# yjh0410/YOLO-Nano

Measured on AMD Instinct MI355X. Metric: images/sec YOLO-Nano-1.0x 416x416 bs=32 inference (network + decode + NMS + host delivery), higher is better.
Workload: dtype f32 (split-f16 MFMA x3, fp32 accumulate); 1 GPU; YOLO-Nano-1.0x 416x416 bs=32/GPU fp32 inference, COCO 80-class head + NMS (BASELINE configs[1]); inputs resident in HBM, kept detections delivered to pinned host memory inside the timed region; global_batch=32, parallelism=image-sharded x1, no collective, rccl_ranks=1, launch_mode=eager, streams_per_gpu=4

## Files before the change

### yolo-nano_amd/csrc/kernels_conv.hip

```cpp
#include "yn_internal.h"
#include "yn_device.h"

#include <cstdio>
#include <mutex>
#include <set>
#include <string>

namespace ynk {

static thread_local const char* g_last_kernel = "";
const char* last_kernel_name() { return g_last_kernel; }
void set_last_kernel_name(const char* n) { g_last_kernel = n; }

bool g_log_lds = getenv("YN_LOG_LDS") != nullptr && atoi(getenv("YN_LOG_LDS")) != 0;
void note_launch_lds(const char* kernel, size_t dyn_lds, unsigned threads)
{
    static std::mutex mu;
    static std::set<std::string> seen;
    char line[512];
    snprintf(line, sizeof line, "yn_lds %s %zu %u", kernel, dyn_lds, threads);
    std::lock_guard<std::mutex> lk(mu);
    if (seen.insert(line).second) fprintf(stderr, "%s\n", line);
}

// ... 1008 lines not shown
static int choose_pw_cfg(int M, int K, int Npad)
{
    const int nt32 = Npad / 32;
    auto pick_nt = [&](int wn, int maxnt) {
        const int need = (nt32 + wn - 1) / wn;
        if (need <= maxnt) return need;
        for (int nt = maxnt; nt >= 1; --nt) if (nt32 % (nt * wn) == 0) return nt;
        return maxnt;
    };
    auto blocks = [&](int wm, int wn, int nt) {
        const long BM = 32 * wm, BN = 32 * nt * wn;
        return ((M + BM - 1) / BM) * ((Npad + BN - 1) / BN);
    };
    int wm = 4, wn = 1, nt = pick_nt(1, 4);
    if (blocks(wm, wn, nt) < 384) {
        const int nt2 = pick_nt(2, 2);
        if (blocks(2, 2, nt2) > blocks(wm, wn, nt)) { wm = 2; wn = 2; nt = nt2; }
        if (blocks(wm, wn, nt) < 256) {
            const int nt3 = pick_nt(4, 2);
            if (blocks(1, 4, nt3) > blocks(wm, wn, nt)) { wm = 1; wn = 4; nt = nt3; }
            if (blocks(wm, wn, nt) < 256 && nt > 1 && blocks(wm, wn, 1) > blocks(wm, wn, nt)) nt = 1;
        }
    }
    const bool one_shot = K <= 64;
    int idx = find_pw_cfg(wm, wn, nt, one_shot ? 32 : 16, one_shot ? 1 : 2);
    const TileCfg& c = g_pw_cfgs[idx];
    if (c.WM != wm || c.WN != wn || c.NT != nt) idx = find_pw_cfg(wm, wn, nt, 16, 2);
    return idx;
}

void launch_pw(const GemmArgs& a, hipStream_t s)
{
    int idx = a.cfg;
    if (idx == N_PW_CFGS + N_PWD_CFGS + N_PWS_CFGS) { if (launch_pw_pipe(a, s)) return; idx = -1; }
    if (a.Wsh && (idx < 0 || idx >= N_PW_CFGS + N_PWD_CFGS) && launch_pw_split(a, idx < 0 ? -1 : idx - N_PW_CFGS - N_PWD_CFGS, s)) return;
    if (idx >= N_PW_CFGS + N_PWD_CFGS) idx = -1;
    if (idx >= N_PW_CFGS && idx < N_PW_CFGS + N_PWD_CFGS && launch_pw_direct(a, idx - N_PW_CFGS, s)) return;
    if (idx < 0 || idx >= N_PW_CFGS) idx = choose_pw_cfg(a.M, a.K, a.Npad);
    const TileCfg& c = g_pw_cfgs[idx];
    const int BM = 32 * c.WM, BN = 32 * c.NT * c.WN;
    dim3 grid(xcd_grid((a.M + BM - 1) / BM) * ((a.Npad + BN - 1) / BN));
    g_last_kernel = g_pw_names[idx];
    int i = 0;
#define X(wm, wn, nt, kp, nb)                                                                              \
    if (i++ == idx) { hipLaunchKernelGGL((gemm_conv_kernel<wm, wn, nt, 0, kp, nb>), grid, dim3(256), 0, s, a); return; }
    YN_PW_CONFIGS(X)
#undef X
}

static void launch_gemm_3x3(const GemmArgs& a, hipStream_t s)
{
    const int nt32 = a.Npad / 32;
    if (nt32 % 3 == 0) {
        dim3 grid(xcd_grid((a.M + 127) / 128) * (a.Npad / 96));
        g_last_kernel = "gemm_conv_kernel<4,1,3,1,16,2>";
        hipLaunchKernelGGL((gemm_conv_kernel<4, 1, 3, 1, 16, 2>), grid, dim3(256), 0, s, a);
    } else {
        dim3 grid(xcd_grid((a.M + 127) / 128) * nt32);
        g_last_kernel = "gemm_conv_kernel<4,1,1,1,16,2>";
        hipLaunchKernelGGL((gemm_conv_kernel<4, 1, 1, 1, 16, 2>), grid, dim3(256), 0, s, a);
    }
}

void launch_conv3x3(const GemmArgs& a, hipStream_t s)
{
    const int nt32 = a.Npad / 32;
    const int NT = nt32 >= 3 && nt32 % 3 == 0 ? 3 : (nt32 % 2 == 0 ? 2 : 1);
    if (a.Wsh && a.Wsl && a.K == 96 && a.Npad == 96 && a.in_off == 0 && a.in_ld == 96 && (a.N & 3) == 0 && (a.out_ld & 3) == 0 && (a.out_off & 3) == 0 &&
        conv3x3_split_lds(a.W, 1, 1) <= 160 * 1024) {
        static unsigned long long attr_s = 0;
        if (attr_pending(attr_s)) {
            (void)hipFuncSetAttribute(reinterpret_cast<const void*>(conv3x3_split_kernel<3, 2>), hipFuncAttributeMaxDynamicSharedMemorySize, 160 * 1024);
            (void)hipFuncSetAttribute(reinterpret_cast<const void*>(conv3x3_split_kernel<1, 2, 1>), hipFuncAttributeMaxDynamicSharedMemorySize, 160 * 1024);
            (void)hipFuncSetAttribute(reinterpret_cast<const void*>(conv3x3_split_kernel<1, 1, 9>), hipFuncAttributeMaxDynamicSharedMemorySize, 160 * 1024);
            (void)hipFuncSetAttribute(reinterpret_cast<const void*>(conv3x3_split_kernel<1, 1, 3>), hipFuncAttributeMaxDynamicSharedMemorySize, 160 * 1024);
            (void)hipFuncSetAttribute(reinterpret_cast<const void*>(conv3x3_split_kernel<1, 1, 1>), hipFuncAttributeMaxDynamicSharedMemorySize, 160 * 1024);
        }
        const int tiles = (a.M + 127) / 128;
        if (tiles >= 256) {
            g_last_kernel = "conv3x3_split_kernel<3,2>";
            hipLaunchKernelGGL((conv3x3_split_kernel<3, 2>), dim3(xcd_grid(tiles), 1), dim3(256), conv3x3_split_lds(a.W, 3, 2), s, a);
        } else if (tiles * 3 >= 256) {
            g_last_kernel = "conv3x3_split_kernel<1,2>";
            hipLaunchKernelGGL((conv3x3_split_kernel<1, 2, 1>), dim3(xcd_grid(tiles), 3), dim3(256), conv3x3_split_lds(a.W, 1, 2, 1), s, a);
        } else if (conv3x3_split_lds(a.W, 1, 1, 9) <= 160 * 1024) {
            g_last_kernel = "conv3x3_split_kernel<1,1,9>";
            hipLaunchKernelGGL((conv3x3_split_kernel<1, 1, 9>), dim3(xcd_grid(tiles), 3), dim3(256), conv3x3_split_lds(a.W, 1, 1, 9), s, a);
        } else if (conv3x3_split_lds(a.W, 1, 1, 3) <= 160 * 1024) {
            g_last_kernel = "conv3x3_split_kernel<1,1,3>";
            hipLaunchKernelGGL((conv3x3_split_kernel<1, 1, 3>), dim3(xcd_grid(tiles), 3), dim3(256), conv3x3_split_lds(a.W, 1, 1, 3), s, a);
        } else {
            g_last_kernel = "conv3x3_split_kernel<1,1,1>";
            hipLaunchKernelGGL((conv3x3_split_kernel<1, 1, 1>), dim3(xcd_grid(tiles), 3), dim3(256), conv3x3_split_lds(a.W, 1, 1, 1), s, a);
        }
        return;
    }
    if (a.K == 96 && NT == 3 && a.in_off == 0 && a.in_ld == 96 && (a.N & 3) == 0 && (a.out_ld & 3) == 0 && (a.out_off & 3) == 0 &&
        conv3x3_halo_tap_lds(a.W, 96, 3) <= 160 * 1024) {
        static unsigned long long attr_t = 0;
        if (attr_pending(attr_t)) {
            (void)hipFuncSetAttribute(reinterpret_cast<const void*>(conv3x3_halo_tap_kernel<3, 96, 1>), hipFuncAttributeMaxDynamicSharedMemorySize, 160 * 1024);
            (void)hipFuncSetAttribute(reinterpret_cast<const void*>(conv3x3_halo_tap_kernel<1, 96, 1>), hipFuncAttributeMaxDynamicSharedMemorySize, 160 * 1024);
            (void)hipFuncSetAttribute(reinterpret_cast<const void*>(conv3x3_halo_tap_kernel<1, 96, 2>), hipFuncAttributeMaxDynamicSharedMemorySize, 160 * 1024);
        }
        const int tiles = (a.M + 127) / 128;
        if (tiles * (a.Npad / 96) >= 256) {
            g_last_kernel = "conv3x3_halo_tap_kernel<3,96,1>";
            hipLaunchKernelGGL((conv3x3_halo_tap_kernel<3, 96, 1>), dim3(xcd_grid(tiles), a.Npad / 96), dim3(256), conv3x3_halo_tap_lds(a.W, 96, 3), s, a);
        } else if (conv3x3_halo_tap_lds(a.W, 96, 1) > 80 * 1024 && conv3x3_halo_tap_lds(a.W, 96, 1, 2) <= 80 * 1024) {
            g_last_kernel = "conv3x3_halo_tap_kernel<1,96,2>";
            hipLaunchKernelGGL((conv3x3_halo_tap_kernel<1, 96, 2>), dim3(xcd_grid(tiles), a.Npad / 32), dim3(256), conv3x3_halo_tap_lds(a.W, 96, 1, 2), s, a);
        } else {
            g_last_kernel = "conv3x3_halo_tap_kernel<1,96,1>";
            hipLaunchKernelGGL((conv3x3_halo_tap_kernel<1, 96, 1>), dim3(xcd_grid(tiles), a.Npad / 32), dim3(256), conv3x3_halo_tap_lds(a.W, 96, 1), s, a);
        }
        return;
    }
    const size_t lds = (a.K % 32 == 0 && a.in_off == 0) ? conv3x3_halo_lds(a.W, a.K, NT) : (size_t)1 << 30;
    if (lds <= 160 * 1024 && a.K / 2 <= 256) {
        static unsigned long long attr = 0;
        if (attr_pending(attr)) {
            (void)hipFuncSetAttribute(reinterpret_cast<const void*>(conv3x3_halo_kernel<1>), hipFuncAttributeMaxDynamicSharedMemorySize, 160 * 1024);
            (void)hipFuncSetAttribute(reinterpret_cast<const void*>(conv3x3_halo_kernel<2>), hipFuncAttributeMaxDynamicSharedMemorySize, 160 * 1024);
            (void)hipFuncSetAttribute(reinterpret_cast<const void*>(conv3x3_halo_kernel<3>), hipFuncAttributeMaxDynamicSharedMemorySize, 160 * 1024);
        }
        dim3 grid((a.M + 127) / 128, a.Npad / (32 * NT));
        if (NT == 3) { g_last_kernel = "conv3x3_halo_kernel<3>"; hipLaunchKernelGGL(conv3x3_halo_kernel<3>, grid, dim3(256), lds, s, a); }
        else if (NT == 2) { g_last_kernel = "conv3x3_halo_kernel<2>"; hipLaunchKernelGGL(conv3x3_halo_kernel<2>, grid, dim3(256), lds, s, a); }
        else { g_last_kernel = "conv3x3_halo_kernel<1>"; hipLaunchKernelGGL(conv3x3_halo_kernel<1>, grid, dim3(256), lds, s, a); }
        return;
    }
    launch_gemm_3x3(a, s);
}

template <int STRIDE, int VEC, int R>
__device__ __forceinline__ void dwconv3x3_block(const DwArgs& a, unsigned bid, unsigned nblocks)
{
    typedef typename VecT<VEC>::type vec;
    constexpr int NCOL = STRIDE == 1 ? R + 2 : 2 * R + 1;
    const int Ho = (a.H - 1) / STRIDE + 1, Wo = (a.W - 1) / STRIDE + 1;
    const int cv_n = a.C / VEC, segs = (Wo + R - 1) / R;
    const int total = a.B * Ho * segs * cv_n;
    const int i = xcd_block(bid, nblocks) * 256 + threadIdx.x;
    if (i >= total) return;
    const int cv = i % cv_n;
    int q = i / cv_n;
    const int seg = q % segs; q /= segs;
    const int oy = q % Ho, b = q / Ho;
    const int c = cv * VEC, ox0 = seg * R;
    vec col[3][NCOL];
#pragma unroll
    for (int ky = 0; ky < 3; ++ky) {
        const int iy = oy * STRIDE - 1 + ky;
        const bool yok = iy >= 0 && iy < a.H;
        const float* row = a.in + ((size_t)(b * a.H + (yok ? iy : 0)) * a.W) * a.in_ld + a.in_off + c;
#pragma unroll
        for (int j = 0; j < NCOL; ++j) {
            const int ix = ox0 * STRIDE - 1 + j;
            const unsigned mk = opaque_mask(yok && ix >= 0 && ix < a.W);
            col[ky][j] = vmask(*reinterpret_cast<const vec*>(row + (size_t)(ix < 0 ? 0 : (ix >= a.W ? a.W - 1 : ix)) * a.in_ld), mk);
        }
    }
    vec w[9];
#pragma unroll
    for (int k = 0; k < 9; ++k) w[k] = *reinterpret_cast<const vec*>(a.w + k * a.C + c);
    const vec bias = *reinterpret_cast<const vec*>(a.bias + c);
    float* orow = a.out + ((size_t)(b * Ho + oy) * Wo) * a.out_ld + a.out_off + c;
#pragma unroll
    for (int o = 0; o < R; ++o) {
        if (ox0 + o >= Wo) break;
        vec acc = bias;
#pragma unroll
        for (int ky = 0; ky < 3; ++ky)
#pragma unroll
            for (int kx = 0; kx < 3; ++kx) vfma(acc, col[ky][o * STRIDE + kx], w[ky * 3 + kx]);
        *reinterpret_cast<vec*>(orow + (size_t)(ox0 + o) * a.out_ld) = vact(acc, a.act);
    }
}

template <int STRIDE, int VEC, int R>
__global__ __launch_bounds__(256) void dwconv3x3_kernel(DwArgs a) { dwconv3x3_block<STRIDE, VEC, R>(a, blockIdx.x, gridDim.x); }

template <int R>
__global__ __launch_bounds__(256) void dwconv3x3_group_kernel(Group<DwArgs> g)
{
    unsigned local, nb;
    const int p = group_problem(g.first, blockIdx.x, local, nb);
    dwconv3x3_block<1, 4, R>(g.a[p], local, nb);
}

bool dw_group_ok(const DwArgs* a, int n)
{
    if (n < 1 || n > YN_GROUP_MAX) return false;
    for (int p = 0; p < n; ++p)
        if (a[p].stride != 1 || (a[p].C % 4) || (a[p].in_ld % 4) || (a[p].in_off % 4) || (a[p].out_ld % 4) || (a[p].out_off % 4)) return false;
    return true;
}

void launch_dw_group(const DwArgs* a, int n, hipStream_t s)
{
    auto blocks_for = [&](const DwArgs& q, int r) { return (unsigned)(((long)q.B * q.H * ((q.W + r - 1) / r) * (q.C / 4) + 255) / 256); };
    unsigned all4 = 0;
    for (int p = 0; p < n; ++p) all4 += blocks_for(a[p], 4);
    const int R = all4 >= 1024 ? 4 : 2;
    Group<DwArgs> g{};
    unsigned tot = 0;
    for (int p = 0; p < YN_GROUP_MAX; ++p) {
        g.first[p] = tot;
        if (p < n) { g.a[p] = a[p]; tot += xcd_grid(blocks_for(a[p], R)); }
    }
    g.first[YN_GROUP_MAX] = tot;
    if (R == 4) { g_last_kernel = "dwconv3x3_group_kernel<4>"; hipLaunchKernelGGL(dwconv3x3_group_kernel<4>, dim3(tot), dim3(256), 0, s, g); }
    else        { g_last_kernel = "dwconv3x3_group_kernel<2>"; hipLaunchKernelGGL(dwconv3x3_group_kernel<2>, dim3(tot), dim3(256), 0, s, g); }
}

void launch_dw(const DwArgs& a, hipStream_t s)
{
    const int Ho = (a.H - 1) / a.stride + 1, Wo = (a.W - 1) / a.stride + 1;
    const bool v4 = (a.C % 4 == 0) && (a.in_ld % 4 == 0) && (a.in_off % 4 == 0) && (a.out_ld % 4 == 0) && (a.out_off % 4 == 0);
    auto blocks_for = [&](int vec, int r) { return ((long)a.B * Ho * ((Wo + r - 1) / r) * (a.C / vec) + 255) / 256; };
#define YN_DW(ST, V, R) { g_last_kernel = "dwconv3x3_kernel<" #ST "," #V "," #R ">"; \
        hipLaunchKernelGGL((dwconv3x3_kernel<ST, V, R>), dim3(xcd_grid((unsigned)blocks_for(V, R))), dim3(256), 0, s, a); return; }
    if (a.stride == 1) {
        if (v4) { if (blocks_for(4, 4) >= 1024) YN_DW(1, 4, 4) else YN_DW(1, 4, 2) }
        else    { if (blocks_for(2, 8) >= 1024) YN_DW(1, 2, 8) else YN_DW(1, 2, 4) }
    } else {
        if (v4) { if (blocks_for(4, 4) >= 1024) YN_DW(2, 4, 4) else YN_DW(2, 4, 2) }
        else    { if (blocks_for(2, 4) >= 1024) YN_DW(2, 2, 4) else YN_DW(2, 2, 2) }
    }
#undef YN_DW
}

template <int COUT>
__global__ __launch_bounds__(256) void stem_kernel(const float* __restrict__ x, int B, int H, int W,
                                                    const float* __restrict__ w, const float* __restrict__ bias,
                                                    int act, float* __restrict__ y)
{
    __shared__ __attribute__((aligned(16))) float ws[28 * COUT];
    for (int i = threadIdx.x; i < 27 * COUT; i += 256) ws[i] = w[i];
    for (int i = threadIdx.x; i < COUT; i += 256) ws[27 * COUT + i] = bias[i];
    __syncthreads();
    const int Ho = (H - 1) / 2 + 1, Wo = (W - 1) / 2 + 1, Wp = (Wo + 1) / 2;
    const long total = (long)B * Ho * Wp;
    const long p = (long)blockIdx.x * 256 + threadIdx.x;
    if (p >= total) return;
    const int opx = (int)(p % Wp);
    const long q = p / Wp;
    const int oy = (int)(q % Ho);
    const int b = (int)(q / Ho);
    const int ox0 = opx * 2;
    const bool has1 = ox0 + 1 < Wo;
    float acc0[COUT], acc1[COUT];
#pragma unroll
    for (int co = 0; co < COUT; ++co) { acc0[co] = ws[27 * COUT + co]; acc1[co] = acc0[co]; }
#pragma unroll 1
    for (int cy = 0; cy < 9; ++cy) {
        const int ci = cy / 3, ky = cy - ci * 3;
        const float* xp = x + ((size_t)b * 3 + ci) * H * W;
        {
            const int iy = oy * 2 - 1 + ky;
            const bool rowok = iy >= 0 && iy < H;
            float in[5];
#pragma unroll
            for (int j = 0; j < 5; ++j) {
                const int ix = ox0 * 2 - 1 + j;
                in[j] = (rowok && ix >= 0 && ix < W) ? xp[(size_t)iy * W + ix] : 0.0f;
            }
#pragma unroll
            for (int kx = 0; kx < 3; ++kx) {
                const float4* wr = reinterpret_cast<const float4*>(ws + ((ci * 3 + ky) * 3 + kx) * COUT);
#pragma unroll
                for (int c4 = 0; c4 < COUT / 4; ++c4) {
                    const float4 wv = wr[c4];
                    acc0[c4 * 4 + 0] += in[kx] * wv.x; acc0[c4 * 4 + 1] += in[kx] * wv.y;
                    acc0[c4 * 4 + 2] += in[kx] * wv.z; acc0[c4 * 4 + 3] += in[kx] * wv.w;
                    acc1[c4 * 4 + 0] += in[kx + 2] * wv.x; acc1[c4 * 4 + 1] += in[kx + 2] * wv.y;
                    acc1[c4 * 4 + 2] += in[kx + 2] * wv.z; acc1[c4 * 4 + 3] += in[kx + 2] * wv.w;
                }
            }
        }
    }
    float* yo = y + (((size_t)b * Ho + oy) * Wo + ox0) * COUT;
#pragma unroll
    for (int co = 0; co < COUT; co += 4)
        *reinterpret_cast<float4*>(yo + co) = make_float4(apply_act(acc0[co], act), apply_act(acc0[co + 1], act),
                                                          apply_act(acc0[co + 2], act), apply_act(acc0[co + 3], act));
    if (has1) {
#pragma unroll
        for (int co = 0; co < COUT; co += 4)
            *reinterpret_cast<float4*>(yo + COUT + co) = make_float4(apply_act(acc1[co], act), apply_act(acc1[co + 1], act),
                                                                     apply_act(acc1[co + 2], act), apply_act(acc1[co + 3], act));
    }
}

void launch_stem(const float* x, int B, int H, int W, const float* w, const float* bias, int Cout, int act, float* y, hipStream_t s)
{
    const int Ho = (H - 1) / 2 + 1, Wo = (W - 1) / 2 + 1;
    const long total = (long)B * Ho * ((Wo + 1) / 2);
    const unsigned blocks = (unsigned)((total + 255) / 256);
    g_last_kernel = "stem_kernel<24>";
    if (Cout == 24) hipLaunchKernelGGL(stem_kernel<24>, dim3(blocks), dim3(256), 0, s, x, B, H, W, w, bias, act, y);
}

template <int COUT>
__global__ __launch_bounds__(256) void stem_pool_kernel(const float* __restrict__ x, int B, int H, int W,
                                                         const float* __restrict__ w, const float* __restrict__ bias,
                                                         int act, float* __restrict__ y)
{
    constexpr int PR = 8, PC = 7, CR = 2 * PR + 1, CC = 2 * PC + 1;
    __shared__ __attribute__((aligned(16))) float ct[CR * CC * COUT];
    const int Hc = (H - 1) / 2 + 1, Wc = (W - 1) / 2 + 1;
    const int Hp = (Hc - 1) / 2 + 1, Wp = (Wc - 1) / 2 + 1;
    const int tiles_x = (Wp + PC - 1) / PC, tiles_y = (Hp + PR - 1) / PR;
    const int vb = (int)xcd_block(blockIdx.x, gridDim.x);
    if (vb >= tiles_x * tiles_y * B) return;
    const int tile = vb % (tiles_x * tiles_y), b = vb / (tiles_x * tiles_y);
    const int py0 = (tile / tiles_x) * PR, px0 = (tile % tiles_x) * PC;
    const int t = threadIdx.x;
    const int r = t / CC, c = t - r * CC;
    const int cy = 2 * py0 - 1 + r, cx = 2 * px0 - 1 + c;
    const bool live = t < CR * CC && cy >= 0 && cy < Hc && cx >= 0 && cx < Wc;
    float in[27];
    {
        const int cyc = live ? cy : 0, cxc = live ? cx : 0;
#pragma unroll
        for (int q = 0; q < 9; ++q) {
            const int ci = q / 3, ky = q - ci * 3;
            const float* xp = x + ((size_t)b * 3 + ci) * H * W;
            const int iy = cyc * 2 - 1 + ky;
            const bool rowok = live && iy >= 0 && iy < H;
            const float* xr = xp + (size_t)(iy < 0 ? 0 : (iy >= H ? H - 1 : iy)) * W;
#pragma unroll
            for (int k = 0; k < 3; ++k) {
                const int ix = cxc * 2 - 1 + k;
                const unsigned mk = opaque_mask(rowok && ix >= 0 && ix < W);
                in[q * 3 + k] = __uint_as_float(__float_as_uint(xr[ix < 0 ? 0 : (ix >= W ? W - 1 : ix)]) & mk);
            }
        }
    }
    float acc[COUT];
#pragma unroll
    for (int co = 0; co < COUT; ++co) acc[co] = bias[co];
#pragma unroll
    for (int i = 0; i < 27; ++i) {
#pragma unroll
        for (int co = 0; co < COUT; ++co) acc[co] += in[i] * w[i * COUT + co];
    }
#pragma unroll
    for (int co = 0; co < COUT; ++co) acc[co] = live ? apply_act(acc[co], act) : -INFINITY;
    if (t < CR * CC) {
#pragma unroll
        for (int co = 0; co < COUT; co += 4)
            *reinterpret_cast<float4*>(ct + t * COUT + co) = make_float4(acc[co], acc[co + 1], acc[co + 2], acc[co + 3]);
    }
    __syncthreads();
    constexpr int C4 = COUT / 4;
    for (int i = t; i < PR * PC * C4; i += 256) {
        const int c4 = i % C4, pp = i / C4;
        const int pr = pp / PC, pc = pp - pr * PC;
        const int py = py0 + pr, px = px0 + pc;
        if (py >= Hp || px >= Wp) continue;
        float4 m = make_float4(-INFINITY, -INFINITY, -INFINITY, -INFINITY);
#pragma unroll
        for (int dy = 0; dy < 3; ++dy)
#pragma unroll
            for (int dx = 0; dx < 3; ++dx) {
                const float4 v = *reinterpret_cast<const float4*>(ct + ((2 * pr + dy) * CC + 2 * pc + dx) * COUT + c4 * 4);
                m.x = fmaxf(m.x, v.x); m.y = fmaxf(m.y, v.y); m.z = fmaxf(m.z, v.z); m.w = fmaxf(m.w, v.w);
            }
        *reinterpret_cast<float4*>(y + (((size_t)b * Hp + py) * Wp + px) * COUT + c4 * 4) = m;
    }
}

void launch_stem_pool(const float* x, int B, int H, int W, const float* w, const float* bias, int Cout, int act, float* y, hipStream_t s)
{
    const int Hc = (H - 1) / 2 + 1, Wc = (W - 1) / 2 + 1, Hp = (Hc - 1) / 2 + 1, Wp = (Wc - 1) / 2 + 1;
    const int tiles = ((Wp + 6) / 7) * ((Hp + 7) / 8);
    g_last_kernel = "stem_pool_kernel<24>";
    if (Cout == 24) hipLaunchKernelGGL(stem_pool_kernel<24>, dim3(xcd_grid((unsigned)(tiles * B))), dim3(256), 0, s, x, B, H, W, w, bias, act, y);
}

__global__ __launch_bounds__(256) void maxpool_kernel(const float* __restrict__ x, int B, int H, int W, int C, float* __restrict__ y)
{
    const int Ho = (H - 1) / 2 + 1, Wo = (W - 1) / 2 + 1;
    const int c4n = C >> 2;
    const long total = (long)B * Ho * Wo * c4n;
    for (long i = (long)blockIdx.x * 256 + threadIdx.x; i < total; i += (long)gridDim.x * 256) {
        const int c4 = (int)(i % c4n);
        const long p = i / c4n;
        const int ox = (int)(p % Wo);
        const long q = p / Wo;
        const int oy = (int)(q % Ho);
        const int b = (int)(q / Ho);
        float4 m = make_float4(-INFINITY, -INFINITY, -INFINITY, -INFINITY);
#pragma unroll
        for (int ky = 0; ky < 3; ++ky) {
            const int iy = oy * 2 - 1 + ky;
            if (iy < 0 || iy >= H) continue;
#pragma unroll
            for (int kx = 0; kx < 3; ++kx) {
                const int ix = ox * 2 - 1 + kx;
                if (ix < 0 || ix >= W) continue;
                const float4 v = *reinterpret_cast<const float4*>(x + ((size_t)(b * H + iy) * W + ix) * C + c4 * 4);
                m.x = fmaxf(m.x, v.x); m.y = fmaxf(m.y, v.y); m.z = fmaxf(m.z, v.z); m.w = fmaxf(m.w, v.w);
            }
        }
        *reinterpret_cast<float4*>(y + (size_t)p * C + c4 * 4) = m;
    }
}

void launch_maxpool(const float* x, int B, int H, int W, int C, float* y, hipStream_t s)
{
    const int Ho = (H - 1) / 2 + 1, Wo = (W - 1) / 2 + 1;
    const long total = (long)B * Ho * Wo * (C >> 2);
    long blocks = (total + 255) / 256;
    if (blocks > 256 * 32) blocks = 256 * 32;
    if (blocks < 1) blocks = 1;
    g_last_kernel = "maxpool_kernel";
    hipLaunchKernelGGL(maxpool_kernel, dim3((unsigned)blocks), dim3(256), 0, s, x, B, H, W, C, y);
}

__global__ void nchw_to_nhwc_kernel(const float* __restrict__ x, int B, int C, int HW, float* __restrict__ y)
{
    __shared__ float tile[32][33];
    const int b = blockIdx.z;
    const int p0 = blockIdx.x * 32, c0 = blockIdx.y * 32;
    const int tx = threadIdx.x & 31, ty = threadIdx.x >> 5;
    for (int r = ty; r < 32; r += 8) {
        const int c = c0 + r, p = p0 + tx;
        tile[r][tx] = (c < C && p < HW) ? x[((size_t)b * C + c) * HW + p] : 0.0f;
    }
    __syncthreads();
    for (int r = ty; r < 32; r += 8) {
        const int p = p0 + r, c = c0 + tx;
        if (p < HW && c < C) y[((size_t)b * HW + p) * C + c] = tile[tx][r];
    }
}

void launch_nchw_to_nhwc(const float* x, int B, int C, int H, int W, float* y, hipStream_t s)
{
    const int HW = H * W;
    dim3 grid((HW + 31) / 32, (C + 31) / 32, B);
    hipLaunchKernelGGL(nchw_to_nhwc_kernel, grid, dim3(256), 0, s, x, B, C, HW, y);
}

void launch_nhwc_to_nchw(const float* x, int B, int C, int H, int W, float* y, hipStream_t s)
{
    const int HW = H * W;
    dim3 grid((C + 31) / 32, (HW + 31) / 32, B);
    hipLaunchKernelGGL(nchw_to_nhwc_kernel, grid, dim3(256), 0, s, x, B, HW, C, y);
}

__global__ void fold_pack_kernel(FoldArgs a)
{
    const int per_out = (a.kind == 1) ? a.kk : a.Cin * a.kk;
    const int total = a.Cout * per_out;
    const int i = blockIdx.x * 256 + threadIdx.x;
    if (i < a.Cout) {
        const int co = i;
        float f = 1.0f, bv = a.b ? a.b[co] : 0.0f;
        if (a.gamma) {
            f = a.gamma[co] / sqrtf(a.var[co] + a.eps);
            bv = (bv - a.mean[co]) * f + a.beta[co];
        }
        if (a.b_ref) a.b_ref[co] = bv;
        a.b_packed[co] = bv;
    }
    if (i >= total) return;
    const int co = i / per_out, r = i - co * per_out;
    float f = 1.0f;
    if (a.gamma) f = a.gamma[co] / sqrtf(a.var[co] + a.eps);
    const float v = a.w[i] * f;
    if (a.w_ref) a.w_ref[i] = v;
    if (a.kind == 1) {
        a.w_packed[r * a.Cout + co] = v;
    } else if (a.kind == 2) {
        a.w_packed[r * a.Cout + co] = v;
    } else {
        const int ci = r / a.kk, tap = r - ci * a.kk;
        const int k = tap * a.Cin + ci;
        a.w_packed[((size_t)(k >> 1) * a.Npad + co) * 2 + (k & 1)] = v;
        if (a.ws_hi) {
            if (a.w_ovf && !(fabsf(v) < 65504.0f)) atomicOr(a.w_ovf, 1u);
            const _Float16 hi = (_Float16)v, lo = split_lo(v, hi);
            const size_t o = (((size_t)tap * ((a.Cin + 7) >> 3) + (ci >> 3)) * a.Npad + co) * 8 + (ci & 7);
            reinterpret_cast<_Float16*>(a.ws_hi)[o] = hi;
            reinterpret_cast<_Float16*>(a.ws_lo)[o] = lo;
        }
    }
}

void launch_fold_pack(const FoldArgs& a, hipStream_t s)
{
    const int per_out = (a.kind == 1) ? a.kk : a.Cin * a.kk;
    int total = a.Cout * per_out;
    if (total < a.Cout) total = a.Cout;
    hipLaunchKernelGGL(fold_pack_kernel, dim3((total + 255) / 256), dim3(256), 0, s, a);
}

}
```

Before: 51340 images/s.

## Specialize stem+pool kernel for interior tiles with scalar-loaded pipelined weights

Splits the fused stem conv + maxpool kernel into an interior-tile path with no bounds checks and a boundary path that masks after loading. Weights are streamed through double-buffered inline-asm scalar loads (s_load_dwordx8) so they come from SGPRs instead of per-lane loads. The FMA uses packed float2 vector FMAs. A launch-bounds occupancy hint of 6 is added. The bit-exact special case, a rounded mul-add on one channel for later inputs, looks like matching the reference's rounding, and the inline asm wait/clobber constraints are fragile.

```diff
diff --git a/yolo-nano_amd/csrc/kernels_conv.hip b/yolo-nano_amd/csrc/kernels_conv.hip
--- a/yolo-nano_amd/csrc/kernels_conv.hip
+++ b/yolo-nano_amd/csrc/kernels_conv.hip
@@ -1334,13 +1334,133 @@
     if (Cout == 24) hipLaunchKernelGGL(stem_kernel<24>, dim3(blocks), dim3(256), 0, s, x, B, H, W, w, bias, act, y);
 }
 
+struct StemPoolGeom { static constexpr int PR = 8, PC = 7, CR = 2 * PR + 1, CC = 2 * PC + 1; };
+typedef float stem_f4 __attribute__((ext_vector_type(4)));
+typedef float stem_f2 __attribute__((ext_vector_type(2)));
+typedef float stem_f8 __attribute__((ext_vector_type(8)));
+
+__device__ __forceinline__ void stem_w_issue(const float* w, stem_f8 (&q)[3], float& v)
+{
+    asm volatile("s_load_dwordx8 %0, %4, 0x0\n\ts_load_dwordx8 %1, %4, 0x20\n\ts_load_dwordx8 %2, %4, 0x40"
+                 : "=&s"(q[0]), "=&s"(q[1]), "=&s"(q[2]), "+v"(v) : "s"(w));
+}
+__device__ __forceinline__ void stem_w_wait(stem_f8 (&q)[3], stem_f2 (&a)[12])
+{
+    asm volatile("s_waitcnt lgkmcnt(0)" : "+s"(q[0]), "+s"(q[1]), "+s"(q[2]), "+v"(a[0]), "+v"(a[1]), "+v"(a[2]), "+v"(a[3]), "+v"(a[4]), "+v"(a[5]),
+                                          "+v"(a[6]), "+v"(a[7]), "+v"(a[8]), "+v"(a[9]), "+v"(a[10]), "+v"(a[11]));
+}
+
+__device__ __forceinline__ float stem_mul_add_rounded(float a, float b, float c)
+{
+#pragma clang fp contract(off)
+    const float p = a * b;
+    return c + p;
+}
+
+template <int COUT, bool INNER>
+__device__ __forceinline__ void stem_pool_tile(stem_f4* ct, const float* __restrict__ x, int b, int py0, int px0, int H, int W,
+                                               const float* __restrict__ w, const float* __restrict__ bias, int act, float* __restrict__ y)
+{
+    constexpr int PR = StemPoolGeom::PR, PC = StemPoolGeom::PC, CR = StemPoolGeom::CR, CC = StemPoolGeom::CC;
+    constexpr int C4 = COUT / 4;
+    const int Hc = (H - 1) / 2 + 1, Wc = (W - 1) / 2 + 1;
+    const int Hp = (Hc - 1) / 2 + 1, Wp = (Wc - 1) / 2 + 1;
+    const int t = threadIdx.x;
+    const int tp = INNER && t >= CR * CC ? CR * CC - 1 : t;
+    const int r = tp / CC, c = tp - r * CC;
+    const int cy = 2 * py0 - 1 + r, cx = 2 * px0 - 1 + c;
+    const bool live = INNER || (t < CR * CC && cy >= 0 && cy < Hc && cx >= 0 && cx < Wc);
+    float in[27];
+    bool ok[27];
+    if (INNER) {
+        const float* xt = x + (size_t)b * 3 * H * W + ((size_t)(cy * 2 - 1) * W + (cx * 2 - 1));
+#pragma unroll
+        for (int q = 0; q < 9; ++q) {
+            const int ci = q / 3, ky = q - ci * 3;
+            const float* xr = xt + ((size_t)ci * H + ky) * W;
+#pragma unroll
+            for (int k = 0; k < 3; ++k) in[q * 3 + k] = xr[k];
+        }
+    } else {
+        const int cyc = live ? cy : 0, cxc = live ? cx : 0;
+#pragma unroll
+        for (int q = 0; q < 9; ++q) {
+            const int ci = q / 3, ky = q - ci * 3;
+            const float* xp = x + ((size_t)b * 3 + ci) * H * W;
+            const int iy = cyc * 2 - 1 + ky;
+            const bool rowok = live && iy >= 0 && iy < H;
+            const float* xr = xp + (size_t)(iy < 0 ? 0 : (iy >= H ? H - 1 : iy)) * W;
+#pragma unroll
+            for (int k = 0; k < 3; ++k) {
+                const int ix = cxc * 2 - 1 + k;
+                ok[q * 3 + k] = rowok && ix >= 0 && ix < W;
+                in[q * 3 + k] = xr[ix < 0 ? 0 : (ix >= W ? W - 1 : ix)];
+            }
+        }
+    }
+    asm volatile("" : "+v"(in[0]), "+v"(in[1]), "+v"(in[2]), "+v"(in[3]), "+v"(in[4]), "+v"(in[5]), "+v"(in[6]), "+v"(in[7]), "+v"(in[8]),
+                      "+v"(in[9]), "+v"(in[10]), "+v"(in[11]), "+v"(in[12]), "+v"(in[13]), "+v"(in[14]), "+v"(in[15]), "+v"(in[16]), "+v"(in[17]),
+                      "+v"(in[18]), "+v"(in[19]), "+v"(in[20]), "+v"(in[21]), "+v"(in[22]), "+v"(in[23]), "+v"(in[24]), "+v"(in[25]), "+v"(in[26]));
+    if (!INNER) {
+#pragma unroll
+        for (int i = 0; i < 27; ++i) in[i] = ok[i] ? in[i] : 0.0f;
+    }
+    static_assert(COUT == 24, "the weight stream is written for three 8-weight scalar loads per input");
+    stem_f2 acc[COUT / 2];
+#pragma unroll
+    for (int p = 0; p < COUT / 2; ++p) acc[p] = stem_f2{bias[2 * p], bias[2 * p + 1]};
+    stem_f8 wq[2][3];
+    stem_w_issue(w, wq[0], in[0]);
+#pragma unroll
+    for (int i = 0; i < 27; ++i) {
+        stem_w_wait(wq[i & 1], acc);
+        if (i + 1 < 27) stem_w_issue(w + (i + 1) * COUT, wq[(i + 1) & 1], in[i]);
+        const stem_f2 v = {in[i], in[i]};
+#pragma unroll
+        for (int p = 0; p < COUT / 2; ++p) {
+            const stem_f8 w8 = wq[i & 1][p / 4];
+            const stem_f2 f = __builtin_elementwise_fma(v, stem_f2{w8[2 * (p % 4)], w8[2 * (p % 4) + 1]}, acc[p]);
+            acc[p] = (p == 0 && i >= 15) ? stem_f2{stem_mul_add_rounded(in[i], w8[0], acc[0].x), f.y} : f;
+        }
+    }
+    float out[COUT];
+#pragma unroll
+    for (int co = 0; co < COUT; ++co) out[co] = live ? apply_act(co & 1 ? acc[co / 2].y : acc[co / 2].x, act) : -INFINITY;
+    if (t < CR * CC) {
+#pragma unroll
+        for (int c4 = 0; c4 < C4; ++c4)
+            ct[t * C4 + c4] = stem_f4{out[c4 * 4], out[c4 * 4 + 1], out[c4 * 4 + 2], out[c4 * 4 + 3]};
+    }
+    __syncthreads();
+    constexpr int ITEMS = PR * PC * C4;
+    auto pool = [&](int i) {
+        const int c4 = i % C4, pp = i / C4;
+        const int pr = pp / PC, pc = pp - pr * PC;
+        const stem_f4* s = ct + (2 * pr * CC + 2 * pc) * C4 + c4;
+        stem_f4 m = {-INFINITY, -INFINITY, -INFINITY, -INFINITY};
+#pragma unroll
+        for (int k = 0; k < 9; ++k) {
+            const stem_f4 v = s[((k / 3) * CC + k % 3) * C4];
+            m.x = fmaxf(m.x, v.x); m.y = fmaxf(m.y, v.y); m.z = fmaxf(m.z, v.z); m.w = fmaxf(m.w, v.w);
+        }
+        return m;
+    };
+    auto put = [&](int i, stem_f4 m) {
+        const int c4 = i % C4, pp = i / C4;
+        const int pr = pp / PC, pc = pp - pr * PC;
+        const int py = py0 + pr, px = px0 + pc;
+        if (INNER || (py < Hp && px < Wp)) *reinterpret_cast<stem_f4*>(y + (((size_t)b * Hp + py) * Wp + px) * COUT + c4 * 4) = m;
+    };
+    for (int i = t; i < ITEMS; i += 256) put(i, pool(i));
+}
+
 template <int COUT>
-__global__ __launch_bounds__(256) void stem_pool_kernel(const float* __restrict__ x, int B, int H, int W,
+__global__ __launch_bounds__(256, 6) void stem_pool_kernel(const float* __restrict__ x, int B, int H, int W,
                                                          const float* __restrict__ w, const float* __restrict__ bias,
                                                          int act, float* __restrict__ y)
 {
-    constexpr int PR = 8, PC = 7, CR = 2 * PR + 1, CC = 2 * PC + 1;
-    __shared__ __attribute__((aligned(16))) float ct[CR * CC * COUT];
+    constexpr int PR = StemPoolGeom::PR, PC = StemPoolGeom::PC, CR = StemPoolGeom::CR, CC = StemPoolGeom::CC;
+    __shared__ stem_f4 ct[CR * CC * (COUT / 4)];
     const int Hc = (H - 1) / 2 + 1, Wc = (W - 1) / 2 + 1;
     const int Hp = (Hc - 1) / 2 + 1, Wp = (Wc - 1) / 2 + 1;
     const int tiles_x = (Wp + PC - 1) / PC, tiles_y = (Hp + PR - 1) / PR;
@@ -1348,60 +1468,9 @@
     if (vb >= tiles_x * tiles_y * B) return;
     const int tile = vb % (tiles_x * tiles_y), b = vb / (tiles_x * tiles_y);
     const int py0 = (tile / tiles_x) * PR, px0 = (tile % tiles_x) * PC;
-    const int t = threadIdx.x;
-    const int r = t / CC, c = t - r * CC;
-    const int cy = 2 * py0 - 1 + r, cx = 2 * px0 - 1 + c;
-    const bool live = t < CR * CC && cy >= 0 && cy < Hc && cx >= 0 && cx < Wc;
-    float in[27];
-    {
-        const int cyc = live ? cy : 0, cxc = live ? cx : 0;
-#pragma unroll
-        for (int q = 0; q < 9; ++q) {
-            const int ci = q / 3, ky = q - ci * 3;
-            const float* xp = x + ((size_t)b * 3 + ci) * H * W;
-            const int iy = cyc * 2 - 1 + ky;
-            const bool rowok = live && iy >= 0 && iy < H;
-            const float* xr = xp + (size_t)(iy < 0 ? 0 : (iy >= H ? H - 1 : iy)) * W;
-#pragma unroll
-            for (int k = 0; k < 3; ++k) {
-                const int ix = cxc * 2 - 1 + k;
-                const unsigned mk = opaque_mask(rowok && ix >= 0 && ix < W);
-                in[q * 3 + k] = __uint_as_float(__float_as_uint(xr[ix < 0 ? 0 : (ix >= W ? W - 1 : ix)]) & mk);
-            }
-        }
-    }
-    float acc[COUT];
-#pragma unroll
-    for (int co = 0; co < COUT; ++co) acc[co] = bias[co];
-#pragma unroll
-    for (int i = 0; i < 27; ++i) {
-#pragma unroll
-        for (int co = 0; co < COUT; ++co) acc[co] += in[i] * w[i * COUT + co];
-    }
-#pragma unroll
-    for (int co = 0; co < COUT; ++co) acc[co] = live ? apply_act(acc[co], act) : -INFINITY;
-    if (t < CR * CC) {
-#pragma unroll
-        for (int co = 0; co < COUT; co += 4)
-            *reinterpret_cast<float4*>(ct + t * COUT + co) = make_float4(acc[co], acc[co + 1], acc[co + 2], acc[co + 3]);
-    }
-    __syncthreads();
-    constexpr int C4 = COUT / 4;
-    for (int i = t; i < PR * PC * C4; i += 256) {
-        const int c4 = i % C4, pp = i / C4;
-        const int pr = pp / PC, pc = pp - pr * PC;
-        const int py = py0 + pr, px = px0 + pc;
-        if (py >= Hp || px >= Wp) continue;
-        float4 m = make_float4(-INFINITY, -INFINITY, -INFINITY, -INFINITY);
-#pragma unroll
-        for (int dy = 0; dy < 3; ++dy)
-#pragma unroll
-            for (int dx = 0; dx < 3; ++dx) {
-                const float4 v = *reinterpret_cast<const float4*>(ct + ((2 * pr + dy) * CC + 2 * pc + dx) * COUT + c4 * 4);
-                m.x = fmaxf(m.x, v.x); m.y = fmaxf(m.y, v.y); m.z = fmaxf(m.z, v.z); m.w = fmaxf(m.w, v.w);
-            }
-        *reinterpret_cast<float4*>(y + (((size_t)b * Hp + py) * Wp + px) * COUT + c4 * 4) = m;
-    }
+    const bool inner = py0 > 0 && px0 > 0 && 4 * py0 + 2 * CR - 3 < H && 4 * px0 + 2 * CC - 3 < W;
+    if (inner) stem_pool_tile<COUT, true>(ct, x, b, py0, px0, H, W, w, bias, act, y);
+    else       stem_pool_tile<COUT, false>(ct, x, b, py0, px0, H, W, w, bias, act, y);
 }
 
 void launch_stem_pool(const float* x, int B, int H, int W, const float* w, const float* bias, int Cout, int act, float* y, hipStream_t s)
```

Result: no change. 51800 images/s (median of 6 runs) (+0.9%).
